# danijar/crafter

Measured on AMD Instinct MI355X. Metric: env-steps/sec (whole node), random policy, 4096 envs, higher is better.
Workload: dtype u8/i32 (+f64 render filters)

## Files before the change

__graft_entry__.py:

```python
import pathlib
import sys

ROOT = pathlib.Path(__file__).resolve().parent
if str(ROOT) not in sys.path:
  sys.path.insert(0, str(ROOT))


def build():
  from crafter_amd import build as hip_build
  path = hip_build.build()
  print(f'[build] {path}')
  from oracle import noise
  print(f'[build] {noise.build()}')
  from tests.hostsim import build as hostsim_build
  print(f'[build] {hostsim_build.build()}')
  from tests.hostsim import symbolic_build
  print(f'[build] {symbolic_build.build()}')
  from tests.hostsim import final_build
  print(f'[build] {final_build.build()}')
  from tests.hostsim import levels_build
  print(f'[build] {levels_build.build()}')
  from tests.hostsim import subset_build
  print(f'[build] {subset_build.build()}')
  from tests.hostsim import levelset_build
  print(f'[build] {levelset_build.build()}')
  from tests.hostsim import worlds_build
  print(f'[build] {worlds_build.build()}')
  import crafter_amd
  from crafter_amd import lib
  lib.load()
  print('[build] crafter_amd imported, libcrafter_hip.so loaded, ABI', lib.load().crafter_abi_version())


def smoke():
  import numpy as np
  import torch
  from crafter_amd import BatchedEnv
  from oracle.crafter_oracle import OracleEnv
  from tests.parity import assert_same
  assert torch.cuda.is_available(), 'smoke() needs a GPU'
  seeds = [1000, 1001, 1002, 1003]
  env = BatchedEnv(len(seeds), seeds=seeds, device='cuda:0', auto_reset=False, semantic=True)
  orcs = [OracleEnv(seed=s) for s in seeds]
  obs = env.reset().cpu().numpy()
  for i, o in enumerate(orcs):
    assert np.array_equal(obs[i], o.reset()), f'reset obs env {i}'
  rs = np.random.RandomState(0)
  for t in range(30):
    acts = rs.randint(0, 17, size=len(seeds)).astype(np.int32)
    obs, rew, done, info = env.step(torch.from_numpy(acts).to('cuda:0'))
# ... 16 lines not shown
```

crafter_amd/csrc/crafter_hip.hip:

```cpp
#include <hip/hip_runtime.h>
#include <hip/hip_ext.h>
#include <stdio.h>
#include <stdlib.h>
#include <string.h>

#include <map>
#include <mutex>
#include <string>
#include <vector>

#include "../../include/crafter_hip.h"
#include "crafter_rollout.hpp"
#include "crafter_subset.hpp"
#include "dispatch_order.hpp"
#include "env_copy.hpp"
#include "env_kernels.hpp"
#include "env_levels.hpp"
#include "env_worlds.hpp"
#include "launch_plan.hpp"
#include "legal.hpp"
#include "symbolic.hpp"
#include "wave_gfx950.hpp"

using namespace crafter;

namespace {

constexpr int kResetThreads = 1024;
constexpr int kRequeueGrid = 256;
constexpr int kRequeueGridPooled = 8;
constexpr int kGenSeedThreads = 64;
constexpr int kGenClassifyThreads = 256;
constexpr int kGenResolveThreads = 64;
constexpr int kGenSerialGrid = 2048;
constexpr int kGenClassifyGridStep = 304;
constexpr int kGenClassifyGrid = 256;
constexpr int kDefaultGenPeriod = 16;
constexpr int kUnpooledStretch = 16;
constexpr int kGenRing = 8;
constexpr int kGenLag = 3;
constexpr int kGenStreams = 2;
constexpr int kMaxLds = 160 * 1024;

template <int LM, int GEO, int RUL>
#ifndef CRAFTER_BIG_WAVES
#define CRAFTER_BIG_WAVES 6
#endif
__global__ void __launch_bounds__(kStepThreads, LM == 0 ? CRAFTER_BIG_WAVES : 1)
crafter_step_kernel(Config cfg_in, TablePtrs tb, StatePtrs st, const int32_t* __restrict__ actions,
                    uint8_t* __restrict__ obs, float* __restrict__ reward, uint8_t* __restrict__ done,
                    StepCtl ctl) {
  extern __shared__ __attribute__((aligned(16))) uint8_t smem[];
  typedef WaveGfx950<kStepThreads> WS;
  WS w;
  const Config cfg = GEO == 1 ? with_default_geometry(cfg_in) : GEO == 2 ? with_default_view(cfg_in) : cfg_in;
  int env = (int)blockIdx.x;
  if (ctl.order_build) {
    if (env == 0) {
      build_order(cfg, tb, ctl.order_build, ctl.next_step, (uint32_t*)smem);
      return;
    }
    env -= 1;
    if (ctl.order) env = ctl.order[env];
  }
// ... 363 lines not shown
static uint64_t mix64(uint64_t h, const void* p, size_t n) {
  const uint8_t* b = (const uint8_t*)p;
  for (size_t i = 0; i < n; i++) {
    h += b[i] + 0x9e3779b97f4a7c15ull;
    h = (h ^ (h >> 30)) * 0xbf58476d1ce4e5b9ull;
    h = (h ^ (h >> 27)) * 0x94d049bb133111ebull;
    h ^= h >> 31;
  }
  return h;
}

struct crafter_handle {
  Config cfg;
  TablePtrs tb;
  StatePtrs st;
  bool have_tables = false;
  bool have_state = false;
  std::vector<void*> owned;
  std::string shared_block_key;
  LaunchPlan plan;
  int gen_resolve_lds_bytes = 0;
  int split = -1;
  int requeue_grid = kRequeueGridPooled;
  int gen_lag = kGenLag;
  int classify_grid = kGenClassifyGrid;
  int classify_grid_step = kGenClassifyGrid;
  long long steps = 0;
  std::string err;
  bool pool = false;
  hipStream_t side[2] = {nullptr, nullptr};
  int32_t* order = nullptr;
  int32_t* next_step = nullptr;
  uint64_t ordered_launches = 0;
  const int32_t* order_override = nullptr;
  int lds_pad = 0;
  int rollout_order = 1;
  int rollout_lds_pad = 0;
  int32_t* stalled_at = nullptr;
  uint32_t* night_px = nullptr;
  uint32_t* noise_raw = nullptr;
  int noise_ahead = 1;
  hipStream_t aux = nullptr;
  int wide = -1;
  hipEvent_t ev_rules = nullptr, ev_requeue = nullptr;
  hipEvent_t ev_main = nullptr;
  int probe_lds[3] = {-1, -1, -1}, probe_big = 0;
  int probe_worlds = 0, probe_us[3] = {80, 120, 300};
  int probe_free_gen = 0;
  int early_frame = -1;
  int gen_classify_prio = 0;
  int gen_serial_prio = -1;
  bool fold_main_event = true;
  hipEvent_t ev_gen[8] = {nullptr, nullptr, nullptr, nullptr, nullptr, nullptr, nullptr, nullptr};
  uint32_t batches = 1;
  uint32_t safe_seq = 1;
  uint32_t polled_seq = 1;
  hipStream_t safe_stream = nullptr;
  bool have_safe_stream = false;
  hipStream_t last_stream = nullptr;
  bool have_last_stream = false;
  hipEvent_t ev_switch = nullptr;
  bool pool_failed = false;
  std::string pool_err;
  int gen_parity = 0;
  int steps_since_gen = 0;
  int gen_period = 8;
  int32_t* copy_mark = nullptr;
  int32_t* copy_verdict = nullptr;
  int32_t copy_stamp = 0;
  LevelTable* levels = nullptr;
  int32_t* subset_actions = nullptr;
  bool timing = false;
  std::vector<hipEvent_t> events;
};

static int fail(crafter_handle* h, const std::string& msg) {
  if (h)
    h->err = msg;
  else
    g_create_error = msg;
  return 1;
}

static int hip_fail(crafter_handle* h, const char* what, hipError_t e) {
  return fail(h, std::string(what) + ": " + hipGetErrorString(e));
}

template <int GEO>
static void launch_generation(crafter_handle* h, hipStream_t side, dim3 gs, dim3 gc, int seg, uint32_t seq, int prio) {
  hipLaunchKernelGGL(crafter_gen_seed_kernel<GEO>, gs, dim3(kGenSeedThreads), kGenSeedLds, side, h->cfg, h->tb, h->st, seg, prio, (const LevelTable*)h->levels);
  hipLaunchKernelGGL(crafter_gen_classify_kernel<GEO>, gc, dim3(kGenClassifyThreads), gen_classify_lds_bytes(h->cfg), side, h->cfg, h->tb, h->st, seg, h->gen_classify_prio);
  hipLaunchKernelGGL(crafter_gen_resolve_kernel<GEO>, gs, dim3(kGenResolveThreads), h->gen_resolve_lds_bytes, side, h->cfg, h->tb,
                     h->st, seg, seq, prio);
}
#ifdef CRAFTER_PROBES
template <int GEO>
static void launch_generation_stamp(crafter_handle* h, hipStream_t side, int seg, uint32_t seq) {
  hipLaunchKernelGGL(crafter_gen_stamp_kernel<GEO>, dim3(64), dim3(kStepThreads), 0, side, h->cfg, h->tb, h->st, seg, seq);
}
#endif

extern "C" {

void crafter_struct_sizes(int32_t out[6]) {
  out[0] = sizeof(Obj);
  out[1] = sizeof(EnvRec);
  out[2] = sizeof(Rules);
  out[3] = sizeof(Config);
  out[4] = sizeof(StatePtrs);
  out[5] = sizeof(TablePtrs);
}

int32_t crafter_abi_version(void) { return 7; }

// ... 7 lines not shown
    return fail(nullptr, "crafter_create: bad view geometry");
  if (c.size_w < 1 || c.size_h < 1 || (long long)c.size_w * c.size_h > (1 << 22))
    return fail(nullptr, "crafter_create: bad image size (at most 2^22 pixels)");
  if (render_static_bytes(c) + sprite_rows_bytes(c) > kRenderStaticBound)
    return fail(nullptr, "crafter_create: image size too large for the renderer's LDS tables (width + height of the view in pixels)");
  int count = 0;
  hipError_t e = hipGetDeviceCount(&count);
  if (e != hipSuccess || count < 1)
    return fail(nullptr, "crafter_create: no HIP device visible (this library has no CPU path)");
  crafter_handle* h = new crafter_handle();
  h->cfg = c;
  if (const char* pad = probe_env("CRAFTER_LDS_PAD")) h->lds_pad = atoi(pad) > 0 ? atoi(pad) : 0;
  if (const char* v = probe_env("CRAFTER_ROLLOUT_ORDER")) h->rollout_order = atoi(v) != 0;
  if (const char* v = probe_env("CRAFTER_FOLD_MAIN_EVENT")) h->fold_main_event = atoi(v) != 0;
  if (const char* v = probe_env("CRAFTER_GEN_SERIAL_PRIO")) h->gen_serial_prio = atoi(v);
  if (const char* v = probe_env("CRAFTER_GEN_CLASSIFY_PRIO")) h->gen_classify_prio = atoi(v);
  if (const char* v = probe_env("CRAFTER_PROBE_FREE_GEN")) h->probe_free_gen = atoi(v);
  if (const char* v = probe_env("CRAFTER_PROBE_OCCUPY_LDS")) sscanf(v, "%d,%d,%d", &h->probe_lds[0], &h->probe_lds[1], &h->probe_lds[2]);
  if (const char* v = probe_env("CRAFTER_PROBE_OCCUPY_BIG")) h->probe_big = atoi(v);
  if (const char* v = probe_env("CRAFTER_PROBE_OCCUPY")) sscanf(v, "%d,%d,%d,%d", &h->probe_worlds, &h->probe_us[0], &h->probe_us[1], &h->probe_us[2]);
  if (const char* pad = probe_env("CRAFTER_ROLLOUT_LDS_PAD")) h->rollout_lds_pad = atoi(pad) > 0 ? atoi(pad) : 0;
  h->plan = launch_plan(c, false, h->lds_pad, h->rollout_lds_pad);
  h->gen_resolve_lds_bytes = gen_resolve_layout(c).total;
  if (const char* v = probe_env("CRAFTER_GEN_LAG")) h->gen_lag = atoi(v) >= 1 && atoi(v) <= kGenRing - 2 ? atoi(v) : kGenLag;
  if (const char* v = getenv("CRAFTER_SPLIT")) h->split = atoi(v) < 0 ? -1 : atoi(v) != 0 ? 1 : 0;
  if (const char* v = probe_env("CRAFTER_NOISE_AHEAD")) h->noise_ahead = atoi(v) != 0;
  if (const char* v = getenv("CRAFTER_STEP_WIDE")) h->wide = atoi(v) != 0 ? 1 : 0;
  if (const char* v = getenv("CRAFTER_STEP_EARLY")) h->early_frame = atoi(v) != 0 ? 1 : 0;
  if (const char* v = probe_env("CRAFTER_REQUEUE_GRID")) h->requeue_grid = atoi(v) >= 1 && atoi(v) <= kRequeueGrid ? atoi(v) : kRequeueGridPooled;
  if (!h->plan.maps_in_lds) h->classify_grid = 2 * kGenClassifyGrid;
  h->classify_grid_step = h->plan.gen_geo ? kGenClassifyGridStep : h->classify_grid;
  if (const char* v = probe_env("CRAFTER_GEN_CLASSIFY_GRID")) h->classify_grid = h->classify_grid_step = atoi(v) > 0 ? atoi(v) : h->classify_grid;
  if (h->plan.render_lds > kMaxLds) {
    std::string msg = "crafter_create: one environment needs " + std::to_string(h->plan.render_lds) +
                      " B of LDS (> 160 KiB): area / max_objects too large for the LDS-resident kernels";
    delete h;
    return fail(nullptr, msg);
  }
  if ((c.step_threads != 0 && c.step_threads != kStepThreads) || (c.reset_threads != 0 && c.reset_threads != kResetThreads)) {
    delete h;
    return fail(nullptr, "crafter_create: workgroup sizes are fixed in this build (step_threads 0 or " +
                             std::to_string(kStepThreads) + ", reset_threads 0 or " + std::to_string(kResetThreads) + ")");
  }
  if (h->plan.opt_in_lds) {
    std::vector<const void*> big;
#define CRAFTER_X(id, LM, GEO, RUL) \
    if constexpr (GEO != 1) big.push_back((const void*)crafter_step_kernel<LM, GEO, RUL>);
// ... 30 lines not shown
    if (keeps_dispatch_order(c.num_envs, v ? atoi(v) : -1)) {
      hipError_t ea = hipMalloc((void**)&h->order, 2 * (size_t)c.num_envs * sizeof(int32_t));
      if (ea == hipSuccess) ea = hipMalloc((void**)&h->next_step, (size_t)c.num_envs * sizeof(int32_t));
      if (ea == hipSuccess) ea = hipMemset(h->next_step, 0, (size_t)c.num_envs * sizeof(int32_t));
      if (ea != hipSuccess) {
        std::string msg = std::string("crafter_create: dispatch order buffers: ") + hipGetErrorString(ea);
        delete h;
        return fail(nullptr, msg);
      }
      h->owned.push_back(h->order);
      h->owned.push_back(h->next_step);
    }
  }
  if (c.auto_reset) {
    if (hipStreamCreateWithFlags(&h->aux, hipStreamNonBlocking) != hipSuccess ||
        hipEventCreateWithFlags(&h->ev_rules, hipEventDisableTiming) != hipSuccess ||
        hipEventCreateWithFlags(&h->ev_requeue, hipEventDisableTiming) != hipSuccess) {
      if (h->aux) (void)hipStreamDestroy(h->aux);
      h->aux = nullptr;
    }
  }
  if (c.auto_reset && c.gen_period >= 0) {
    h->pool = true;
    h->gen_period = c.gen_period > 0 ? c.gen_period : kDefaultGenPeriod;
    int lo = 0, hi = 0;
    (void)hipDeviceGetStreamPriorityRange(&lo, &hi);
    bool ok = hipEventCreateWithFlags(&h->ev_main, hipEventDisableTiming) == hipSuccess;
    for (int i = 0; i < kGenStreams && ok; i++)
      ok = hipStreamCreateWithPriority(&h->side[i], hipStreamNonBlocking, lo) == hipSuccess;
    for (int i = 0; i < kGenRing && ok; i++)
      ok = hipEventCreateWithFlags(&h->ev_gen[i], hipEventDisableTiming) == hipSuccess;
    if (!ok) {
      delete h;
      return fail(nullptr, "crafter_create: cannot create the world-pool stream / events");
    }
  }
  *out = h;
  return 0;
}

void crafter_destroy(crafter_handle* h) {
  if (!h) return;
  for (int i = 0; i < kGenStreams; i++)
    if (h->side[i]) {
      (void)hipStreamSynchronize(h->side[i]);
      (void)hipStreamDestroy(h->side[i]);
    }
// ... 133 lines not shown
    return fail(h, "crafter_bind_state: world pool enabled but pool buffers missing");
  uintptr_t bits = (uintptr_t)s.mat | (uintptr_t)s.objmap | (uintptr_t)s.objs | (uintptr_t)s.mt | (uintptr_t)s.rec;
  if (bits & 15) return fail(h, "crafter_bind_state: state buffers must be 16-byte aligned");
  h->st = s;
  h->have_state = true;
  return 0;
}

int32_t crafter_lds_bytes(const crafter_handle* h) { return h ? h->plan.step_lds : -1; }

int32_t crafter_slot_map_derived(const crafter_handle* h) { return h ? h->plan.maps_in_lds : -1; }

int32_t crafter_step_instance(const crafter_handle* h) { return h ? h->plan.instance : -1; }

static int ready(crafter_handle* h, const char* who) {
  if (!h) return fail(nullptr, std::string(who) + ": null handle");
  if (!h->have_tables) return fail(h, std::string(who) + ": crafter_upload_tables not called");
  if (!h->have_state) return fail(h, std::string(who) + ": crafter_bind_state not called");
  return 0;
}

static void pool_fail(crafter_handle* h, const char* what, hipError_t e) {
  h->pool_failed = true;
  h->pool_err = std::string("world pool disabled (") + what + ": " + hipGetErrorString(e) + "); finished envs regenerate inline";
}

static void pool_adopt_stream(crafter_handle* h, hipStream_t stream) {
  if (!h->pool || h->pool_failed) return;
  if (h->have_safe_stream && h->safe_stream == stream) return;
  if (h->have_safe_stream)
    for (uint32_t s = (h->safe_seq > h->polled_seq + kGenRing ? h->safe_seq - kGenRing : h->polled_seq) + 1; s <= h->safe_seq; s++) {
      hipError_t ew = hipStreamWaitEvent(stream, h->ev_gen[s % kGenRing], 0);
      if (ew != hipSuccess) {
        pool_fail(h, "hipStreamWaitEvent(new launch stream)", ew);
        h->safe_seq = h->polled_seq;
        break;
      }
    }
  h->safe_stream = stream;
  h->have_safe_stream = true;
}

static int adopt_stream(crafter_handle* h, hipStream_t stream) {
  if (h->have_last_stream && h->last_stream != stream) {
    if (!h->ev_switch) {
      hipError_t ec = hipEventCreateWithFlags(&h->ev_switch, hipEventDisableTiming);
      if (ec != hipSuccess) return hip_fail(h, "stream change: hipEventCreate", ec);
    }
    hipError_t e = hipEventRecord(h->ev_switch, h->last_stream);
    if (e == hipSuccess) e = hipStreamWaitEvent(stream, h->ev_switch, 0);
    if (e != hipSuccess) {
      (void)hipGetLastError();
      hipError_t es = hipDeviceSynchronize();
      if (es != hipSuccess) return hip_fail(h, "stream change: ordering the new stream behind the previous one", es);
    }
  }
  h->last_stream = stream;
  h->have_last_stream = true;
  pool_adopt_stream(h, stream);
  return 0;
}

static void pool_schedule(crafter_handle* h, hipStream_t main, int steps = 1, bool main_recorded = false, bool behind_rollout = false) {
  while (h->polled_seq < h->batches) {
    hipError_t q = hipEventQuery(h->ev_gen[(h->polled_seq + 1) % kGenRing]);
    if (q == hipSuccess) {
      h->polled_seq++;
      if (h->safe_seq < h->polled_seq) h->safe_seq = h->polled_seq;
    } else if (q == hipErrorNotReady) {
      break;
    } else {
      return pool_fail(h, "hipEventQuery", q);
    }
  }
  h->steps_since_gen += steps;
  if (h->steps_since_gen < h->gen_period) return;
  uint32_t seq = h->batches + 1;
  if (seq > (uint32_t)h->gen_lag + 1 && h->safe_seq < seq - h->gen_lag) {
    uint32_t t = seq - h->gen_lag;
    hipError_t ew = hipStreamWaitEvent(main, h->ev_gen[t % kGenRing], 0);
    if (ew != hipSuccess) return pool_fail(h, "hipStreamWaitEvent(launch stream)", ew);
    h->safe_seq = t;
  }
  hipStream_t side = h->side[seq % kGenStreams];
  hipError_t e = main_recorded ? hipSuccess : hipEventRecord(h->ev_main, main);
  if (e != hipSuccess) return pool_fail(h, "hipEventRecord(launch stream)", e);
  e = hipStreamWaitEvent(side, h->ev_main, 0);
  if (e != hipSuccess) return pool_fail(h, "hipStreamWaitEvent(generation stream)", e);
  int seg = h->gen_parity;
  int n = h->cfg.num_envs;
  const int prio = h->gen_serial_prio >= 0 ? h->gen_serial_prio : (behind_rollout ? 2 : 1);
  const int cgrid = behind_rollout ? h->classify_grid : h->classify_grid_step;
  dim3 gs(n < kGenSerialGrid ? n : kGenSerialGrid), gc((long long)n * gen_classify_parts(h->cfg) < cgrid ? n * gen_classify_parts(h->cfg) : cgrid);
#ifdef CRAFTER_PROBES
  if (h->probe_free_gen) {
    if (h->probe_free_gen == 2) {
      const int worlds = h->probe_worlds > 0 ? h->probe_worlds : 390;
      int ws = worlds < (int)gs.x ? worlds : (int)gs.x, wc = worlds * gen_classify_parts(h->cfg) < (int)gc.x ? worlds * gen_classify_parts(h->cfg) : (int)gc.x;
      const int l0 = h->probe_lds[0] >= 0 ? h->probe_lds[0] : kGenSeedLds, l1 = h->probe_lds[1] >= 0 ? h->probe_lds[1] : gen_classify_lds_bytes(h->cfg),
                l2 = h->probe_lds[2] >= 0 ? h->probe_lds[2] : h->gen_resolve_lds_bytes;
      if (h->probe_big) {
        hipLaunchKernelGGL(crafter_gen_occupy_kernel<0>, dim3(ws), dim3(kGenSeedThreads), l0, side, h->probe_us[0], worlds, (uint32_t*)nullptr);
        hipLaunchKernelGGL(crafter_gen_occupy_kernel<1>, dim3(wc), dim3(kGenClassifyThreads), l1, side, h->probe_us[1], worlds * gen_classify_parts(h->cfg), (uint32_t*)nullptr);
        hipLaunchKernelGGL(crafter_gen_occupy_kernel<1>, dim3(ws), dim3(kGenResolveThreads), l2, side, h->probe_us[2], worlds, (uint32_t*)nullptr);
      } else {
        hipLaunchKernelGGL(crafter_gen_occupy_kernel<0>, dim3(ws), dim3(kGenSeedThreads), l0, side, h->probe_us[0], worlds, (uint32_t*)nullptr);
        hipLaunchKernelGGL(crafter_gen_occupy_kernel<0>, dim3(wc), dim3(kGenClassifyThreads), l1, side, h->probe_us[1], worlds * gen_classify_parts(h->cfg), (uint32_t*)nullptr);
        hipLaunchKernelGGL(crafter_gen_occupy_kernel<0>, dim3(ws), dim3(kGenResolveThreads), l2, side, h->probe_us[2], worlds, (uint32_t*)nullptr);
      }
    }
    if (h->plan.gen_geo)
      launch_generation_stamp<1>(h, side, seg, seq);
    else
      launch_generation_stamp<0>(h, side, seg, seq);
  } else
#endif
  if (h->plan.gen_geo)
    launch_generation<1>(h, side, gs, gc, seg, seq, prio);
  else
    launch_generation<0>(h, side, gs, gc, seg, seq, prio);
  e = hipGetLastError();
  if (e != hipSuccess) return pool_fail(h, "generation kernel launch", e);
  h->batches = seq;
  h->steps_since_gen = 0;
  h->gen_parity = (seg + 1) % kGenRing;
  e = hipMemsetAsync(h->st.gen_q + (size_t)seg * gen_q_stride(h->cfg), 0, 16, side);
  if (e != hipSuccess) return pool_fail(h, "hipMemsetAsync(request segment)", e);
  e = hipEventRecord(h->ev_gen[seq % kGenRing], side);
  if (e != hipSuccess) return pool_fail(h, "hipEventRecord(generation stream)", e);
}

static void pool_wait_all(crafter_handle* h, hipStream_t stream, const char* what) {
  for (uint32_t s = h->safe_seq + 1; s <= h->batches && !h->pool_failed; s++) {
    hipError_t ew = hipStreamWaitEvent(stream, h->ev_gen[s % kGenRing], 0);
    if (ew != hipSuccess) pool_fail(h, what, ew);
  }
  if (!h->pool_failed) h->safe_seq = h->batches;
}

int crafter_reset(crafter_handle* h, const uint8_t* mask, uint8_t* obs, void* stream) {
  if (ready(h, "crafter_reset")) return 1;
  if (adopt_stream(h, (hipStream_t)stream)) return 1;
  if (h->pool && !h->pool_failed) pool_wait_all(h, (hipStream_t)stream, "hipStreamWaitEvent(reset)");
  hipLaunchKernelGGL(crafter_reset_kernel, dim3(h->cfg.num_envs), dim3(kResetThreads), h->plan.reset_lds,
                     (hipStream_t)stream, h->cfg, h->tb, h->st, mask, (h->pool && !h->pool_failed) ? h->gen_parity : -1, obs,
                     (const LevelTable*)h->levels);
  hipError_t e = hipGetLastError();
  if (e != hipSuccess) return hip_fail(h, "crafter_reset launch", e);
  return 0;
}

int crafter_reset_worlds(crafter_handle* h, const uint8_t* mask, const int32_t* world_id, const uint8_t* bank_mat, const crafter_obj* bank_objs,
                         const int32_t* bank_nobj, const int32_t* bank_inv, int32_t n_worlds, int32_t bank_max_objects, uint8_t* obs,
                         void* stream) {
  if (ready(h, "crafter_reset_worlds")) return 1;
  if (!bank_mat || !bank_objs || !bank_nobj) return fail(h, "crafter_reset_worlds: bank_mat, bank_objs and bank_nobj must not be NULL");
  if (n_worlds < 1) return fail(h, "crafter_reset_worlds: n_worlds must be at least 1");
  if (bank_max_objects < 0) return fail(h, "crafter_reset_worlds: bank_max_objects must not be negative");
  if (((uintptr_t)bank_objs & 15u) != 0) return fail(h, "crafter_reset_worlds: bank_objs must be 16-byte aligned");
  if (adopt_stream(h, (hipStream_t)stream)) return 1;
  if (h->pool && !h->pool_failed) pool_wait_all(h, (hipStream_t)stream, "hipStreamWaitEvent(reset_worlds)");
  WorldBank bank;
  bank.world_id = world_id;
  bank.mat = bank_mat;
  bank.objs = bank_objs;
  bank.nobj = bank_nobj;
  bank.inv = bank_inv;
  bank.n_worlds = n_worlds;
  bank.max_objects = bank_max_objects;
  hipLaunchKernelGGL(crafter_reset_worlds_kernel, dim3(h->cfg.num_envs), dim3(kResetThreads), h->plan.reset_lds, (hipStream_t)stream,
                     h->cfg, h->tb, h->st, mask, bank, (h->pool && !h->pool_failed) ? h->gen_parity : -1, obs,
                     (const LevelTable*)h->levels);
  hipError_t e = hipGetLastError();
  if (e != hipSuccess) return hip_fail(h, "crafter_reset_worlds launch", e);
  return 0;
}

static void pool_quiesce(crafter_handle* h, hipStream_t stream) {
  if (!h->pool || h->pool_failed) return;
  pool_schedule(h, stream, h->gen_period);
  pool_wait_all(h, stream, "hipStreamWaitEvent(copy)");
}

static int index_check_scratch(crafter_handle* h, const char* who, hipStream_t stream, int32_t* stamp) {
  if (!h->copy_mark) {
    hipError_t ea = hipMalloc((void**)&h->copy_mark, ((size_t)h->cfg.num_envs + 1) * sizeof(int32_t));
    if (ea != hipSuccess) return hip_fail(h, who, ea);
    h->owned.push_back(h->copy_mark);
    h->copy_verdict = h->copy_mark + h->cfg.num_envs;
    h->copy_stamp = 0;
  }
  if (h->copy_stamp <= 0 || h->copy_stamp == 0x7fffffff) {
    hipError_t em = hipMemsetAsync(h->copy_mark, 0, (size_t)h->cfg.num_envs * sizeof(int32_t), stream);
    if (em != hipSuccess) return hip_fail(h, who, em);
    h->copy_stamp = 0;
  }
  *stamp = ++h->copy_stamp;
  return 0;
}

static int launch_copy(crafter_handle* h, const char* who, int mode, const CopySide& a, const CopySide& b, const int32_t* sidx,
                       const int32_t* didx, int n, hipStream_t stream, bool pool_rows) {
  CopyPlan plan;
// ... 167 lines not shown
  uint64_t k = h->ordered_launches++;
  ctl.order = k > 0 ? h->order + (size_t)(k & 1) * h->cfg.num_envs : nullptr;
  if (h->order_override) ctl.order = h->order_override;
  ctl.order_build = h->order + (size_t)((k + 1) & 1) * h->cfg.num_envs;
  ctl.next_step = h->next_step;
}

static void launch_step_fused(crafter_handle* h, dim3 grid, hipStream_t stream, hipEvent_t start, hipEvent_t stop, const int32_t* actions,
                              uint8_t* obs, float* reward, uint8_t* done, const StepCtl& ctl) {
  switch (h->plan.instance) {
#define CRAFTER_X(id, LM, GEO, RUL)                                                                                              \
    case id:                                                                                                                     \
      CRAFTER_LAUNCH((crafter_step_kernel<LM, GEO, RUL>), grid, dim3(kStepThreads), h->plan.step_lds, stream, start, stop, h->cfg, \
                     h->tb, h->st, actions, obs, reward, done, ctl);                                                             \
      break;
    CRAFTER_STEP_INSTANCES(CRAFTER_X)
#undef CRAFTER_X
  }
}

static int step_launch(crafter_handle* h, const int32_t* actions, uint8_t* obs, float* reward, uint8_t* done, void* stream,
                       const FinalOut* fin) {
  StepCtl ctl;
  const int pool_parity = (h->pool && !h->pool_failed) ? h->gen_parity : -1;
  ctl.gen_parity = fin ? -1 : pool_parity;
  ctl.safe_seq = h->safe_seq;
  hipEvent_t ev[4] = {nullptr, nullptr, nullptr, nullptr};
  const bool frames = h->cfg.render_obs != 0 && obs != nullptr;
  const bool requeue = h->cfg.auto_reset != 0;
  const StepKernel kernel = choose_step(h->plan, h->cfg.num_envs, frames, h->order != nullptr, h->split, h->wide, h->early_frame);
  const bool ordered = h->order && !is_split(kernel);
  ctl.parity = (int)(h->steps++ & 1);
  ctl.early_frame = step_early_frame(h->cfg.num_envs, h->early_frame);
  if (timing_events(h, ev, "crafter_step: hipEventCreate (timing mode)")) return 1;
  if (frames && !is_split(kernel)) {
    if (need_noise_raw(h, "crafter_step: noise scratch")) return 1;
    ctl.noise_raw = h->noise_raw;
  }
  if (ordered) set_dispatch_order(h, ctl);
  if (kernel == kStepRulesFrame && need_night_px(h, "crafter_step: frame kernel scratch")) return 1;
  if (h->plan.night_px) {
    if (frames && need_night_px(h, "crafter_step: night frame scratch")) return 1;
    ctl.night_px = h->night_px;
  }
  const dim3 grid_n(h->cfg.num_envs + (ordered ? 1 : 0)), block_s(kStepThreads);
  bool beside = false;
  switch (kernel) {
    case kStepRules:
      CRAFTER_LAUNCH(crafter_rules_kernel, grid_n, dim3(kRulesThreads), lane_layout(h->cfg).total, (hipStream_t)stream, ev[0], ev[1],
// ... 59 lines not shown
  if (adopt_stream(h, (hipStream_t)stream)) return 1;
  FinalOut fin;
  fin.obs = h->cfg.render_obs != 0 ? final_obs : nullptr;
  fin.terminated = terminated;
  fin.local = final_local;
  fin.stats = final_stats;
  return step_launch(h, actions, obs, reward, done, stream, &fin);
}

int crafter_step_envs(crafter_handle* h, const int32_t* idx, int32_t n, const int32_t* actions, uint8_t* obs, float* reward, uint8_t* done,
                      void* stream) {
  if (ready(h, "crafter_step_envs")) return 1;
  if (n < 0 || n > h->cfg.num_envs) return fail(h, "crafter_step_envs: n outside 0 .. num_envs");
  if (n == 0) return 0;
  if (!idx) return fail(h, "crafter_step_envs: null index list");
  if (!actions || !reward || !done) return fail(h, "crafter_step_envs: null argument");
  if (adopt_stream(h, (hipStream_t)stream)) return 1;
  if (!h->subset_actions) {
    hipError_t ea = hipMalloc((void**)&h->subset_actions, (size_t)h->cfg.num_envs * sizeof(int32_t));
    if (ea != hipSuccess) return hip_fail(h, "crafter_step_envs: actions scratch", ea);
    h->owned.push_back(h->subset_actions);
  }
  StepCtl ctl;
  ctl.gen_parity = (h->pool && !h->pool_failed) ? h->gen_parity : -1;
  ctl.safe_seq = h->safe_seq;
  ctl.early_frame = 0;
  ctl.next_step = h->next_step;
  const bool frames = h->cfg.render_obs != 0 && obs != nullptr;
  const StepEnvsKernel kernel = choose_step_envs(h->plan, n, frames, h->wide);
  hipEvent_t ev[4] = {nullptr, nullptr, nullptr, nullptr};
  if (frames) {
    if (need_noise_raw(h, "crafter_step_envs: noise scratch")) return 1;
    ctl.noise_raw = h->noise_raw;
  }
  if (h->plan.night_px) {
    if (frames && need_night_px(h, "crafter_step_envs: night frame scratch")) return 1;
    ctl.night_px = h->night_px;
  }
  SubsetCheck chk;
  chk.idx = idx; chk.actions = actions; chk.n = n;
  if (index_check_scratch(h, "crafter_step_envs", (hipStream_t)stream, &chk.stamp)) return 1;
  chk.mark = h->copy_mark; chk.verdict = h->copy_verdict; chk.rec = (EnvRec*)h->st.rec; chk.rows = h->cfg.num_envs;
  chk.scattered = h->subset_actions;
  if (timing_events(h, ev, "crafter_step_envs: hipEventCreate (timing mode)")) return 1;
  ctl.parity = (int)(h->steps++ & 1);
  launch_step_envs_check(chk, (hipStream_t)stream, ev[0], nullptr);
  launch_step_subset(kernel, h->plan.instance, n, (size_t)h->plan.step_lds, (hipStream_t)stream, nullptr, ev[1], h->cfg, h->tb, h->st, idx,
                     h->copy_verdict, h->subset_actions, obs, reward, done, ctl);
// ... 40 lines not shown
  h->events.clear();
  *step_ms = a;
  *reset_ms = b;
  *launches = n;
  return 0;
}

int crafter_step_n(crafter_handle* h, int32_t steps, const int32_t* actions, uint8_t* obs, float* reward, uint8_t* done,
                   void* stream) {
  if (ready(h, "crafter_step_n")) return 1;
  if (!actions || !reward || !done || steps < 1) return fail(h, "crafter_step_n: bad argument");
  if (adopt_stream(h, (hipStream_t)stream)) return 1;
  bool pooled = h->pool && !h->pool_failed;
  if (!h->stalled_at) {
    hipError_t ea = hipMalloc((void**)&h->stalled_at, (size_t)h->cfg.num_envs * sizeof(int32_t));
    if (ea != hipSuccess) return hip_fail(h, "crafter_step_n: hipMalloc", ea);
    h->owned.push_back(h->stalled_at);
  }
  const size_t n = (size_t)h->cfg.num_envs;
  const size_t obs_stride = n * (size_t)h->cfg.size_w * h->cfg.size_h * 3;
  bool requeue = h->cfg.auto_reset != 0;
  for (int done_steps = 0; done_steps < steps;) {
    int left = steps - done_steps;
    int room = pooled ? h->gen_period - h->steps_since_gen : (left < kUnpooledStretch ? left : kUnpooledStretch);
    int T = left < room ? left : (room > 0 ? room : 1);
    const int32_t* a = actions + (size_t)done_steps * n;
    uint8_t* o = obs ? obs + (size_t)done_steps * obs_stride : nullptr;
    float* r = reward + (size_t)done_steps * n;
    uint8_t* d = done + (size_t)done_steps * n;
    StepCtl ctl;
    ctl.parity = (int)(h->steps++ & 1);
    ctl.gen_parity = pooled ? h->gen_parity : -1;
    ctl.safe_seq = h->safe_seq;
    RolloutArgs ra;
    ra.T = T; ra.obs_stride = obs_stride; ra.stalled_at = h->stalled_at;
    hipEvent_t ev[4] = {nullptr, nullptr, nullptr, nullptr};
    if (timing_events(h, ev, "crafter_step_n: hipEventCreate (timing mode)")) return 1;
    if (o && h->cfg.render_obs) {
      if (need_noise_raw(h, "crafter_step_n: noise scratch")) return 1;
      ctl.noise_raw = h->noise_raw;
    }
    if (h->order && h->rollout_order) set_dispatch_order(h, ctl);
    if (h->plan.night_px) {
      if (o && h->cfg.render_obs && need_night_px(h, "crafter_step_n: night frame scratch")) return 1;
      ctl.night_px = h->night_px;
    }
    launch_rollout(h->plan.instance, h->cfg.num_envs, (size_t)h->plan.rollout_lds, (hipStream_t)stream, ev[0], ev[1], h->cfg, h->tb, h->st,
                   a, o, r, d, ctl, ra);
    hipError_t e = hipGetLastError();
    if (e != hipSuccess) return hip_fail(h, "crafter_step_n launch", e);
    const bool batch_follows = pooled && requeue && !h->timing && h->fold_main_event && h->steps_since_gen + T >= h->gen_period;
    if (requeue)
      launch_requeue_rollout(requeue_grid(h, ctl), (size_t)h->plan.render_lds, (hipStream_t)stream, ev[2], batch_follows ? h->ev_main : ev[3], h->cfg, h->tb,
                             h->st, a, o, r, d, ctl, ra, h->levels);
    e = hipGetLastError();
    if (e != hipSuccess) return hip_fail(h, "crafter_step_n (auto-reset) launch", e);
    keep_timing_events(h, ev);
    if (pooled) pool_schedule(h, (hipStream_t)stream, T, batch_follows, true);
    pooled = h->pool && !h->pool_failed;
    done_steps += T;
  }
  return 0;
}

int crafter_debug_set_dispatch_order(crafter_handle* h, const int32_t* order) {
  if (ready(h, "crafter_debug_set_dispatch_order")) return 1;
  if (!h->order) return 2;
  if (order) {
    std::vector<int32_t> host((size_t)h->cfg.num_envs);
    hipError_t e = hipMemcpy(host.data(), order, host.size() * sizeof(int32_t), hipMemcpyDeviceToHost);
    if (e != hipSuccess) return hip_fail(h, "crafter_debug_set_dispatch_order", e);
    std::vector<uint8_t> seen(host.size(), 0);
    for (int32_t v : host) {
      if (v < 0 || v >= h->cfg.num_envs || seen[(size_t)v]) return fail(h, "crafter_debug_set_dispatch_order: not a permutation of the env indices");
// ... 50 lines not shown
  if (!legal) return fail(h, "crafter_legal_actions: null output");
  if (adopt_stream(h, (hipStream_t)stream)) return 1;
  const dim3 grid((unsigned)((h->cfg.num_envs + kLegalEnvs - 1) / kLegalEnvs)), block(kLegalThreads);
  if (h->plan.maps_in_lds)
    hipLaunchKernelGGL(crafter_legal_actions_kernel<0>, grid, block, 0, (hipStream_t)stream, h->cfg, h->tb, h->st, mask, legal);
  else
    hipLaunchKernelGGL(crafter_legal_actions_kernel<1>, grid, block, 0, (hipStream_t)stream, h->cfg, h->tb, h->st, mask, legal);
  hipError_t e = hipGetLastError();
  if (e != hipSuccess) return hip_fail(h, "crafter_legal_actions launch", e);
  return 0;
}

#ifdef CRAFTER_PROBES
int crafter_debug_gen_probe(uint64_t out[32]) {
  if (hipDeviceSynchronize() != hipSuccess) return 1;
  if (hipMemcpyFromSymbol(out, HIP_SYMBOL(g_gen_probe), 32 * sizeof(uint64_t)) != hipSuccess) return 1;
  uint64_t zero[32] = {0};
  return hipMemcpyToSymbol(HIP_SYMBOL(g_gen_probe), zero, sizeof(zero)) == hipSuccess ? 0 : 1;
}
#endif

int crafter_pool_status(const crafter_handle* h, uint32_t* launched, uint32_t* trusted) {
  if (!h) return -1;
  if (launched) *launched = h->batches;
  if (trusted) *trusted = h->safe_seq;
  return !h->pool ? 0 : h->pool_failed ? 2 : 1;
}

const char* crafter_pool_error(const crafter_handle* h) { return h ? h->pool_err.c_str() : ""; }

int crafter_debug_eval(int mode, const uint8_t* perm, const double* x, const double* y, const double* z, double* out,
                       int64_t n, void* stream) {
  if (mode < 0 || mode > 3 || !x || !out || n < 0 || (mode == 0 && (!perm || !y || !z)))
    return fail(nullptr, "crafter_debug_eval: bad argument");
  if (n == 0) return 0;
  long long blocks = (n + kStepThreads - 1) / kStepThreads;
  hipLaunchKernelGGL(crafter_debug_eval_kernel, dim3((unsigned)(blocks < 2048 ? blocks : 2048)), dim3(kStepThreads), 512 + kSimplexLdsBytes, (hipStream_t)stream,
                     perm, x, y, z, out, (long long)n, mode);
  hipError_t e = hipGetLastError();
  if (e != hipSuccess) return hip_fail(nullptr, "crafter_debug_eval launch", e);
  return 0;
}

const char* crafter_last_error(const crafter_handle* h) { return h ? h->err.c_str() : g_create_error.c_str(); }

}

#include <dlfcn.h>
// ... 146 lines not shown
```

Baseline: 66.84 million.

## Split world-pool generation so resolve is deferred to the next batch launch

Pool bookkeeping moves into a small PoolBatches state machine that emits command lists. Generation is split in two: seed/classify launches now, and the resolve, segment clear and event record are deferred until the next generation period when defer_step is set (the default for single-step launches). Step-path generation also gets priority 0 for geo configs with at most 4096 envs. The intent is to spread generation work across step windows so it overlaps the step kernels instead of competing in one burst. In exchange, worlds become available one period later, and the minimum lag clamp now rises to 2.

```diff
diff --git a/__graft_entry__.py b/__graft_entry__.py
--- a/__graft_entry__.py
+++ b/__graft_entry__.py
@@ -26,6 +26,8 @@
   print(f'[build] {levelset_build.build()}')
   from tests.hostsim import worlds_build
   print(f'[build] {worlds_build.build()}')
+  from tests.hostsim import pool_batches_build
+  print(f'[build] {pool_batches_build.build()}')
   import crafter_amd
   from crafter_amd import lib
   lib.load()
diff --git a/crafter_amd/csrc/crafter_hip.hip b/crafter_amd/csrc/crafter_hip.hip
--- a/crafter_amd/csrc/crafter_hip.hip
+++ b/crafter_amd/csrc/crafter_hip.hip
@@ -19,6 +19,7 @@
 #include "env_worlds.hpp"
 #include "launch_plan.hpp"
 #include "legal.hpp"
+#include "pool_batches.hpp"
 #include "symbolic.hpp"
 #include "wave_gfx950.hpp"
 
@@ -35,11 +36,9 @@
 constexpr int kGenSerialGrid = 2048;
 constexpr int kGenClassifyGridStep = 304;
 constexpr int kGenClassifyGrid = 256;
+constexpr int kGenPrio0MaxEnvs = 4096;
 constexpr int kDefaultGenPeriod = 16;
 constexpr int kUnpooledStretch = 16;
-constexpr int kGenRing = 8;
-constexpr int kGenLag = 3;
-constexpr int kGenStreams = 2;
 constexpr int kMaxLds = 160 * 1024;
 
 template <int LM, int GEO, int RUL>
@@ -449,12 +448,12 @@
   int gen_resolve_lds_bytes = 0;
   int split = -1;
   int requeue_grid = kRequeueGridPooled;
-  int gen_lag = kGenLag;
   int classify_grid = kGenClassifyGrid;
   int classify_grid_step = kGenClassifyGrid;
   long long steps = 0;
   std::string err;
   bool pool = false;
+  PoolBatches pb;
   hipStream_t side[2] = {nullptr, nullptr};
   int32_t* order = nullptr;
   int32_t* next_step = nullptr;
@@ -479,9 +478,6 @@
   int gen_serial_prio = -1;
   bool fold_main_event = true;
   hipEvent_t ev_gen[8] = {nullptr, nullptr, nullptr, nullptr, nullptr, nullptr, nullptr, nullptr};
-  uint32_t batches = 1;
-  uint32_t safe_seq = 1;
-  uint32_t polled_seq = 1;
   hipStream_t safe_stream = nullptr;
   bool have_safe_stream = false;
   hipStream_t last_stream = nullptr;
@@ -489,9 +485,6 @@
   hipEvent_t ev_switch = nullptr;
   bool pool_failed = false;
   std::string pool_err;
-  int gen_parity = 0;
-  int steps_since_gen = 0;
-  int gen_period = 8;
   int32_t* copy_mark = nullptr;
   int32_t* copy_verdict = nullptr;
   int32_t copy_stamp = 0;
@@ -514,9 +507,12 @@
 }
 
 template <int GEO>
-static void launch_generation(crafter_handle* h, hipStream_t side, dim3 gs, dim3 gc, int seg, uint32_t seq, int prio) {
+static void launch_seed_classify(crafter_handle* h, hipStream_t side, dim3 gs, dim3 gc, int seg, int prio) {
   hipLaunchKernelGGL(crafter_gen_seed_kernel<GEO>, gs, dim3(kGenSeedThreads), kGenSeedLds, side, h->cfg, h->tb, h->st, seg, prio, (const LevelTable*)h->levels);
   hipLaunchKernelGGL(crafter_gen_classify_kernel<GEO>, gc, dim3(kGenClassifyThreads), gen_classify_lds_bytes(h->cfg), side, h->cfg, h->tb, h->st, seg, h->gen_classify_prio);
+}
+template <int GEO>
+static void launch_resolve(crafter_handle* h, hipStream_t side, dim3 gs, int seg, uint32_t seq, int prio) {
   hipLaunchKernelGGL(crafter_gen_resolve_kernel<GEO>, gs, dim3(kGenResolveThreads), h->gen_resolve_lds_bytes, side, h->cfg, h->tb,
                      h->st, seg, seq, prio);
 }
@@ -570,7 +566,13 @@
   if (const char* pad = probe_env("CRAFTER_ROLLOUT_LDS_PAD")) h->rollout_lds_pad = atoi(pad) > 0 ? atoi(pad) : 0;
   h->plan = launch_plan(c, false, h->lds_pad, h->rollout_lds_pad);
   h->gen_resolve_lds_bytes = gen_resolve_layout(c).total;
-  if (const char* v = probe_env("CRAFTER_GEN_LAG")) h->gen_lag = atoi(v) >= 1 && atoi(v) <= kGenRing - 2 ? atoi(v) : kGenLag;
+  if (const char* v = probe_env("CRAFTER_GEN_LAG")) h->pb.gen_lag = clamp_gen_lag(atoi(v));
+  if (const char* v = probe_env("CRAFTER_GEN_DEFER")) {
+    int s = h->pb.defer_step, r = h->pb.defer_rollout;
+    sscanf(v, "%d,%d", &s, &r);
+    h->pb.defer_step = s != 0;
+    h->pb.defer_rollout = r != 0;
+  }
   if (const char* v = getenv("CRAFTER_SPLIT")) h->split = atoi(v) < 0 ? -1 : atoi(v) != 0 ? 1 : 0;
   if (const char* v = probe_env("CRAFTER_NOISE_AHEAD")) h->noise_ahead = atoi(v) != 0;
   if (const char* v = getenv("CRAFTER_STEP_WIDE")) h->wide = atoi(v) != 0 ? 1 : 0;
@@ -647,7 +649,7 @@
   }
   if (c.auto_reset && c.gen_period >= 0) {
     h->pool = true;
-    h->gen_period = c.gen_period > 0 ? c.gen_period : kDefaultGenPeriod;
+    h->pb.gen_period = c.gen_period > 0 ? c.gen_period : kDefaultGenPeriod;
     int lo = 0, hi = 0;
     (void)hipDeviceGetStreamPriorityRange(&lo, &hi);
     bool ok = hipEventCreateWithFlags(&h->ev_main, hipEventDisableTiming) == hipSuccess;
@@ -827,21 +829,24 @@
 
 static void pool_fail(crafter_handle* h, const char* what, hipError_t e) {
   h->pool_failed = true;
+  pool_failed(h->pb);
   h->pool_err = std::string("world pool disabled (") + what + ": " + hipGetErrorString(e) + "); finished envs regenerate inline";
 }
 
 static void pool_adopt_stream(crafter_handle* h, hipStream_t stream) {
   if (!h->pool || h->pool_failed) return;
   if (h->have_safe_stream && h->safe_stream == stream) return;
-  if (h->have_safe_stream)
-    for (uint32_t s = (h->safe_seq > h->polled_seq + kGenRing ? h->safe_seq - kGenRing : h->polled_seq) + 1; s <= h->safe_seq; s++) {
-      hipError_t ew = hipStreamWaitEvent(stream, h->ev_gen[s % kGenRing], 0);
+  if (h->have_safe_stream) {
+    const PoolCmds cmds = plan_adopt(h->pb);
+    for (int i = 0; i < cmds.n; i++) {
+      hipError_t ew = hipStreamWaitEvent(stream, h->ev_gen[cmds.c[i].slot], 0);
       if (ew != hipSuccess) {
         pool_fail(h, "hipStreamWaitEvent(new launch stream)", ew);
-        h->safe_seq = h->polled_seq;
+        adopt_failed(h->pb);
         break;
       }
     }
+  }
   h->safe_stream = stream;
   h->have_safe_stream = true;
 }
@@ -866,35 +871,14 @@
   return 0;
 }
 
-static void pool_schedule(crafter_handle* h, hipStream_t main, int steps = 1, bool main_recorded = false, bool behind_rollout = false) {
-  while (h->polled_seq < h->batches) {
-    hipError_t q = hipEventQuery(h->ev_gen[(h->polled_seq + 1) % kGenRing]);
-    if (q == hipSuccess) {
-      h->polled_seq++;
-      if (h->safe_seq < h->polled_seq) h->safe_seq = h->polled_seq;
-    } else if (q == hipErrorNotReady) {
-      break;
-    } else {
-      return pool_fail(h, "hipEventQuery", q);
-    }
-  }
-  h->steps_since_gen += steps;
-  if (h->steps_since_gen < h->gen_period) return;
-  uint32_t seq = h->batches + 1;
-  if (seq > (uint32_t)h->gen_lag + 1 && h->safe_seq < seq - h->gen_lag) {
-    uint32_t t = seq - h->gen_lag;
-    hipError_t ew = hipStreamWaitEvent(main, h->ev_gen[t % kGenRing], 0);
-    if (ew != hipSuccess) return pool_fail(h, "hipStreamWaitEvent(launch stream)", ew);
-    h->safe_seq = t;
-  }
-  hipStream_t side = h->side[seq % kGenStreams];
-  hipError_t e = main_recorded ? hipSuccess : hipEventRecord(h->ev_main, main);
-  if (e != hipSuccess) return pool_fail(h, "hipEventRecord(launch stream)", e);
-  e = hipStreamWaitEvent(side, h->ev_main, 0);
-  if (e != hipSuccess) return pool_fail(h, "hipStreamWaitEvent(generation stream)", e);
-  int seg = h->gen_parity;
+static hipError_t pool_generation(crafter_handle* h, const PoolCmd& c) {
+  hipStream_t side = h->side[c.side];
+  const bool behind_rollout = c.behind_rollout != 0, first = c.op == kPoolSeedClassify;
+  const int seg = c.seg;
+  const uint32_t seq = c.seq;
   int n = h->cfg.num_envs;
-  const int prio = h->gen_serial_prio >= 0 ? h->gen_serial_prio : (behind_rollout ? 2 : 1);
+  const int step_prio = h->pb.defer_step && h->plan.gen_geo && n <= kGenPrio0MaxEnvs ? 0 : 1;
+  const int prio = h->gen_serial_prio >= 0 ? h->gen_serial_prio : (behind_rollout ? 2 : step_prio);
   const int cgrid = behind_rollout ? h->classify_grid : h->classify_grid_step;
   dim3 gs(n < kGenSerialGrid ? n : kGenSerialGrid), gc((long long)n * gen_classify_parts(h->cfg) < cgrid ? n * gen_classify_parts(h->cfg) : cgrid);
 #ifdef CRAFTER_PROBES
@@ -904,51 +888,93 @@
       int ws = worlds < (int)gs.x ? worlds : (int)gs.x, wc = worlds * gen_classify_parts(h->cfg) < (int)gc.x ? worlds * gen_classify_parts(h->cfg) : (int)gc.x;
       const int l0 = h->probe_lds[0] >= 0 ? h->probe_lds[0] : kGenSeedLds, l1 = h->probe_lds[1] >= 0 ? h->probe_lds[1] : gen_classify_lds_bytes(h->cfg),
                 l2 = h->probe_lds[2] >= 0 ? h->probe_lds[2] : h->gen_resolve_lds_bytes;
-      if (h->probe_big) {
+      if (first) {
         hipLaunchKernelGGL(crafter_gen_occupy_kernel<0>, dim3(ws), dim3(kGenSeedThreads), l0, side, h->probe_us[0], worlds, (uint32_t*)nullptr);
-        hipLaunchKernelGGL(crafter_gen_occupy_kernel<1>, dim3(wc), dim3(kGenClassifyThreads), l1, side, h->probe_us[1], worlds * gen_classify_parts(h->cfg), (uint32_t*)nullptr);
+        if (h->probe_big)
+          hipLaunchKernelGGL(crafter_gen_occupy_kernel<1>, dim3(wc), dim3(kGenClassifyThreads), l1, side, h->probe_us[1], worlds * gen_classify_parts(h->cfg), (uint32_t*)nullptr);
+        else
+          hipLaunchKernelGGL(crafter_gen_occupy_kernel<0>, dim3(wc), dim3(kGenClassifyThreads), l1, side, h->probe_us[1], worlds * gen_classify_parts(h->cfg), (uint32_t*)nullptr);
+      } else if (h->probe_big) {
         hipLaunchKernelGGL(crafter_gen_occupy_kernel<1>, dim3(ws), dim3(kGenResolveThreads), l2, side, h->probe_us[2], worlds, (uint32_t*)nullptr);
       } else {
-        hipLaunchKernelGGL(crafter_gen_occupy_kernel<0>, dim3(ws), dim3(kGenSeedThreads), l0, side, h->probe_us[0], worlds, (uint32_t*)nullptr);
-        hipLaunchKernelGGL(crafter_gen_occupy_kernel<0>, dim3(wc), dim3(kGenClassifyThreads), l1, side, h->probe_us[1], worlds * gen_classify_parts(h->cfg), (uint32_t*)nullptr);
         hipLaunchKernelGGL(crafter_gen_occupy_kernel<0>, dim3(ws), dim3(kGenResolveThreads), l2, side, h->probe_us[2], worlds, (uint32_t*)nullptr);
       }
     }
-    if (h->plan.gen_geo)
+    if (first) {
+    } else if (h->plan.gen_geo)
       launch_generation_stamp<1>(h, side, seg, seq);
     else
       launch_generation_stamp<0>(h, side, seg, seq);
   } else
 #endif
   if (h->plan.gen_geo)
-    launch_generation<1>(h, side, gs, gc, seg, seq, prio);
+    first ? launch_seed_classify<1>(h, side, gs, gc, seg, prio) : launch_resolve<1>(h, side, gs, seg, seq, prio);
   else
-    launch_generation<0>(h, side, gs, gc, seg, seq, prio);
-  e = hipGetLastError();
-  if (e != hipSuccess) return pool_fail(h, "generation kernel launch", e);
-  h->batches = seq;
-  h->steps_since_gen = 0;
-  h->gen_parity = (seg + 1) % kGenRing;
-  e = hipMemsetAsync(h->st.gen_q + (size_t)seg * gen_q_stride(h->cfg), 0, 16, side);
-  if (e != hipSuccess) return pool_fail(h, "hipMemsetAsync(request segment)", e);
-  e = hipEventRecord(h->ev_gen[seq % kGenRing], side);
-  if (e != hipSuccess) return pool_fail(h, "hipEventRecord(generation stream)", e);
-}
-
-static void pool_wait_all(crafter_handle* h, hipStream_t stream, const char* what) {
-  for (uint32_t s = h->safe_seq + 1; s <= h->batches && !h->pool_failed; s++) {
-    hipError_t ew = hipStreamWaitEvent(stream, h->ev_gen[s % kGenRing], 0);
-    if (ew != hipSuccess) pool_fail(h, what, ew);
-  }
-  if (!h->pool_failed) h->safe_seq = h->batches;
-}
+    first ? launch_seed_classify<0>(h, side, gs, gc, seg, prio) : launch_resolve<0>(h, side, gs, seg, seq, prio);
+  return hipGetLastError();
+}
+
+static void pool_run(crafter_handle* h, hipStream_t main, const PoolCmds& cmds, const char* wait_what = "hipStreamWaitEvent(launch stream)") {
+  for (int i = 0; i < cmds.n; i++) {
+    const PoolCmd& c = cmds.c[i];
+    hipStream_t side = h->side[c.side];
+    hipError_t e = hipSuccess;
+    const char* what = "";
+    switch (c.op) {
+      case kPoolMainWaitGen:
+        what = wait_what;
+        e = hipStreamWaitEvent(main, h->ev_gen[c.slot], 0);
+        break;
+      case kPoolRecordMain:
+        what = "hipEventRecord(launch stream)";
+        e = hipEventRecord(h->ev_main, main);
+        break;
+      case kPoolSideWaitMain:
+        what = "hipStreamWaitEvent(generation stream)";
+        e = hipStreamWaitEvent(side, h->ev_main, 0);
+        break;
+      case kPoolSeedClassify:
+      case kPoolResolve:
+        what = "generation kernel launch";
+        e = pool_generation(h, c);
+        break;
+      case kPoolClearSegment:
+        what = "hipMemsetAsync(request segment)";
+        e = hipMemsetAsync(h->st.gen_q + (size_t)c.seg * gen_q_stride(h->cfg), 0, 16, side);
+        break;
+      case kPoolRecordGen:
+        what = "hipEventRecord(generation stream)";
+        e = hipEventRecord(h->ev_gen[c.slot], side);
+        break;
+    }
+    if (e != hipSuccess) return pool_fail(h, what, e);
+    apply(h->pb, c);
+  }
+}
+
+static void pool_schedule(crafter_handle* h, hipStream_t main, int steps = 1, bool main_recorded = false, bool behind_rollout = false) {
+  while (uint32_t s = poll_next(h->pb)) {
+    hipError_t q = hipEventQuery(h->ev_gen[s % kGenRing]);
+    if (q == hipSuccess) {
+      polled(h->pb);
+    } else if (q == hipErrorNotReady) {
+      break;
+    } else {
+      return pool_fail(h, "hipEventQuery", q);
+    }
+  }
+  if (!pool_due(h->pb, steps)) return;
+  pool_run(h, main, plan_launch(h->pb, main_recorded, behind_rollout));
+}
+
+static void pool_wait_all(crafter_handle* h, hipStream_t stream, const char* what) { pool_run(h, stream, plan_flush(h->pb), what); }
 
 int crafter_reset(crafter_handle* h, const uint8_t* mask, uint8_t* obs, void* stream) {
   if (ready(h, "crafter_reset")) return 1;
   if (adopt_stream(h, (hipStream_t)stream)) return 1;
   if (h->pool && !h->pool_failed) pool_wait_all(h, (hipStream_t)stream, "hipStreamWaitEvent(reset)");
   hipLaunchKernelGGL(crafter_reset_kernel, dim3(h->cfg.num_envs), dim3(kResetThreads), h->plan.reset_lds,
-                     (hipStream_t)stream, h->cfg, h->tb, h->st, mask, (h->pool && !h->pool_failed) ? h->gen_parity : -1, obs,
+                     (hipStream_t)stream, h->cfg, h->tb, h->st, mask, (h->pool && !h->pool_failed) ? h->pb.gen_parity : -1, obs,
                      (const LevelTable*)h->levels);
   hipError_t e = hipGetLastError();
   if (e != hipSuccess) return hip_fail(h, "crafter_reset launch", e);
@@ -974,7 +1000,7 @@
   bank.n_worlds = n_worlds;
   bank.max_objects = bank_max_objects;
   hipLaunchKernelGGL(crafter_reset_worlds_kernel, dim3(h->cfg.num_envs), dim3(kResetThreads), h->plan.reset_lds, (hipStream_t)stream,
-                     h->cfg, h->tb, h->st, mask, bank, (h->pool && !h->pool_failed) ? h->gen_parity : -1, obs,
+                     h->cfg, h->tb, h->st, mask, bank, (h->pool && !h->pool_failed) ? h->pb.gen_parity : -1, obs,
                      (const LevelTable*)h->levels);
   hipError_t e = hipGetLastError();
   if (e != hipSuccess) return hip_fail(h, "crafter_reset_worlds launch", e);
@@ -983,7 +1009,7 @@
 
 static void pool_quiesce(crafter_handle* h, hipStream_t stream) {
   if (!h->pool || h->pool_failed) return;
-  pool_schedule(h, stream, h->gen_period);
+  pool_schedule(h, stream, h->pb.gen_period);
   pool_wait_all(h, stream, "hipStreamWaitEvent(copy)");
 }
 
@@ -1197,9 +1223,9 @@
 static int step_launch(crafter_handle* h, const int32_t* actions, uint8_t* obs, float* reward, uint8_t* done, void* stream,
                        const FinalOut* fin) {
   StepCtl ctl;
-  const int pool_parity = (h->pool && !h->pool_failed) ? h->gen_parity : -1;
+  const int pool_parity = (h->pool && !h->pool_failed) ? h->pb.gen_parity : -1;
   ctl.gen_parity = fin ? -1 : pool_parity;
-  ctl.safe_seq = h->safe_seq;
+  ctl.safe_seq = h->pb.safe_seq;
   hipEvent_t ev[4] = {nullptr, nullptr, nullptr, nullptr};
   const bool frames = h->cfg.render_obs != 0 && obs != nullptr;
   const bool requeue = h->cfg.auto_reset != 0;
@@ -1305,8 +1331,8 @@
     h->owned.push_back(h->subset_actions);
   }
   StepCtl ctl;
-  ctl.gen_parity = (h->pool && !h->pool_failed) ? h->gen_parity : -1;
-  ctl.safe_seq = h->safe_seq;
+  ctl.gen_parity = (h->pool && !h->pool_failed) ? h->pb.gen_parity : -1;
+  ctl.safe_seq = h->pb.safe_seq;
   ctl.early_frame = 0;
   ctl.next_step = h->next_step;
   const bool frames = h->cfg.render_obs != 0 && obs != nullptr;
@@ -1393,7 +1419,7 @@
   bool requeue = h->cfg.auto_reset != 0;
   for (int done_steps = 0; done_steps < steps;) {
     int left = steps - done_steps;
-    int room = pooled ? h->gen_period - h->steps_since_gen : (left < kUnpooledStretch ? left : kUnpooledStretch);
+    int room = pooled ? h->pb.gen_period - h->pb.steps_since_gen : (left < kUnpooledStretch ? left : kUnpooledStretch);
     int T = left < room ? left : (room > 0 ? room : 1);
     const int32_t* a = actions + (size_t)done_steps * n;
     uint8_t* o = obs ? obs + (size_t)done_steps * obs_stride : nullptr;
@@ -1401,8 +1427,8 @@
     uint8_t* d = done + (size_t)done_steps * n;
     StepCtl ctl;
     ctl.parity = (int)(h->steps++ & 1);
-    ctl.gen_parity = pooled ? h->gen_parity : -1;
-    ctl.safe_seq = h->safe_seq;
+    ctl.gen_parity = pooled ? h->pb.gen_parity : -1;
+    ctl.safe_seq = h->pb.safe_seq;
     RolloutArgs ra;
     ra.T = T; ra.obs_stride = obs_stride; ra.stalled_at = h->stalled_at;
     hipEvent_t ev[4] = {nullptr, nullptr, nullptr, nullptr};
@@ -1420,7 +1446,7 @@
                    a, o, r, d, ctl, ra);
     hipError_t e = hipGetLastError();
     if (e != hipSuccess) return hip_fail(h, "crafter_step_n launch", e);
-    const bool batch_follows = pooled && requeue && !h->timing && h->fold_main_event && h->steps_since_gen + T >= h->gen_period;
+    const bool batch_follows = pooled && requeue && !h->timing && h->fold_main_event && h->pb.steps_since_gen + T >= h->pb.gen_period;
     if (requeue)
       launch_requeue_rollout(requeue_grid(h, ctl), (size_t)h->plan.render_lds, (hipStream_t)stream, ev[2], batch_follows ? h->ev_main : ev[3], h->cfg, h->tb,
                              h->st, a, o, r, d, ctl, ra, h->levels);
@@ -1517,8 +1543,8 @@
 
 int crafter_pool_status(const crafter_handle* h, uint32_t* launched, uint32_t* trusted) {
   if (!h) return -1;
-  if (launched) *launched = h->batches;
-  if (trusted) *trusted = h->safe_seq;
+  if (launched) *launched = h->pb.batches;
+  if (trusted) *trusted = h->pb.safe_seq;
   return !h->pool ? 0 : h->pool_failed ? 2 : 1;
 }
 
diff --git a/crafter_amd/csrc/pool_batches.hpp b/crafter_amd/csrc/pool_batches.hpp
--- /dev/null
+++ b/crafter_amd/csrc/pool_batches.hpp
@@ -0,0 +1,133 @@
+#pragma once
+#include <stdint.h>
+
+namespace crafter {
+
+constexpr int kGenRing = 8;
+constexpr int kGenStreams = 2;
+constexpr int kGenLag = 3;
+constexpr int kGenLagMin = 2, kGenLagMax = kGenRing - 3;
+
+inline int clamp_gen_lag(int v) { return v < kGenLagMin ? kGenLagMin : v > kGenLagMax ? kGenLagMax : v; }
+
+enum PoolOp {
+  kPoolMainWaitGen,
+  kPoolRecordMain,
+  kPoolSideWaitMain,
+  kPoolSeedClassify,
+  kPoolResolve,
+  kPoolClearSegment,
+  kPoolRecordGen,
+};
+
+struct PoolCmd {
+  int op;
+  uint32_t seq;
+  int side, seg, slot;
+  int behind_rollout;
+};
+
+struct PoolCmds {
+  int n = 0;
+  PoolCmd c[kGenRing + 10];
+  void add(int op, uint32_t seq, int seg, int behind_rollout) {
+    c[n++] = PoolCmd{op, seq, (int)(seq % kGenStreams), seg, (int)(seq % kGenRing), behind_rollout};
+  }
+};
+
+struct PoolBatches {
+  int gen_lag = kGenLag;
+  int gen_period = 8;
+  int defer_step = 1;
+  int defer_rollout = 0;
+  uint32_t batches = 1;
+  uint32_t pending = 0;
+  int pending_seg = 0, pending_rollout = 0;
+  uint32_t safe_seq = 1;
+  uint32_t polled_seq = 1;
+  int gen_parity = 0;
+  int steps_since_gen = 0;
+  bool failed = false;
+};
+
+inline uint32_t poll_next(const PoolBatches& b) { return !b.failed && b.polled_seq < b.batches ? b.polled_seq + 1 : 0; }
+inline void polled(PoolBatches& b) {
+  b.polled_seq++;
+  if (b.safe_seq < b.polled_seq) b.safe_seq = b.polled_seq;
+}
+
+inline bool pool_due(PoolBatches& b, int steps) {
+  b.steps_since_gen += steps;
+  return !b.failed && b.steps_since_gen >= b.gen_period;
+}
+
+inline void add_remainder(PoolCmds& out, uint32_t seq, int seg, int behind_rollout) {
+  out.add(kPoolResolve, seq, seg, behind_rollout);
+  out.add(kPoolClearSegment, seq, seg, behind_rollout);
+  out.add(kPoolRecordGen, seq, seg, behind_rollout);
+}
+
+inline PoolCmds plan_launch(const PoolBatches& b, bool main_recorded, bool behind_rollout) {
+  PoolCmds out;
+  if (b.failed) return out;
+  const uint32_t seq = (b.pending ? b.pending : b.batches) + 1;
+  if (seq > (uint32_t)b.gen_lag + 1 && b.safe_seq < seq - b.gen_lag) out.add(kPoolMainWaitGen, seq - b.gen_lag, 0, 0);
+  if (!main_recorded) out.add(kPoolRecordMain, seq, 0, 0);
+  if (b.pending) {
+    out.add(kPoolSideWaitMain, b.pending, b.pending_seg, b.pending_rollout);
+    add_remainder(out, b.pending, b.pending_seg, b.pending_rollout);
+  }
+  out.add(kPoolSideWaitMain, seq, b.gen_parity, behind_rollout);
+  out.add(kPoolSeedClassify, seq, b.gen_parity, behind_rollout);
+  if (!(behind_rollout ? b.defer_rollout : b.defer_step)) add_remainder(out, seq, b.gen_parity, behind_rollout);
+  return out;
+}
+
+inline PoolCmds plan_flush(const PoolBatches& b) {
+  PoolCmds out;
+  if (b.failed) return out;
+  if (b.pending) add_remainder(out, b.pending, b.pending_seg, b.pending_rollout);
+  const uint32_t last = b.pending ? b.pending : b.batches;
+  for (uint32_t s = (last > b.safe_seq + kGenRing ? last - kGenRing : b.safe_seq) + 1; s <= last; s++) out.add(kPoolMainWaitGen, s, 0, 0);
+  return out;
+}
+
+inline PoolCmds plan_adopt(const PoolBatches& b) {
+  PoolCmds out;
+  if (b.failed) return out;
+  for (uint32_t s = (b.safe_seq > b.polled_seq + kGenRing ? b.safe_seq - kGenRing : b.polled_seq) + 1; s <= b.safe_seq; s++)
+    out.add(kPoolMainWaitGen, s, 0, 0);
+  return out;
+}
+
+inline void apply(PoolBatches& b, const PoolCmd& c) {
+  switch (c.op) {
+    case kPoolMainWaitGen:
+      if (b.safe_seq < c.seq) b.safe_seq = c.seq;
+      break;
+    case kPoolSeedClassify:
+      b.pending = c.seq;
+      b.pending_seg = c.seg;
+      b.pending_rollout = c.behind_rollout;
+      b.steps_since_gen = 0;
+      b.gen_parity = (c.seg + 1) % kGenRing;
+      break;
+    case kPoolRecordGen:
+      b.batches = c.seq;
+      b.pending = 0;
+      break;
+    default:
+      break;
+  }
+}
+
+inline void pool_failed(PoolBatches& b) {
+  b.failed = true;
+  b.pending = 0;
+}
+inline void adopt_failed(PoolBatches& b) {
+  pool_failed(b);
+  b.safe_seq = b.polled_seq;
+}
+
+}
```

Result: slower. 65.73 million (-1.7%).
